# jfjlaros/HUMID

Measured on AMD Instinct MI355X. Metric: reads/sec deduplicated, 10M PE150 UMI=8 d=1, higher is better.
Workload: dtype u64; 1 GPU; 10000000 reads/GPU x 1 GPU (one shuffled read set of 10000000 reads, sliced by input order), PE150 UMI=8 in header -> 24-nt packed words (8+8+8), d=1, directional clustering; synthetic molecules=N/4, family 1+Geom(3), p_sub=1e-3, p_N=1e-4; reads_per_gpu=10000000, word_nt=24, distance=1, method=directional

## Files before the change

humid_amd/_lib.py:

```python
from __future__ import annotations

import ctypes as C
import os

_HERE = os.path.dirname(os.path.abspath(__file__))
SO_PATH = os.path.join(_HERE, "libhumid_hip.so")

u64p = C.POINTER(C.c_uint64)
u32p = C.POINTER(C.c_uint32)
u8p = C.POINTER(C.c_uint8)


class HumidSummary(C.Structure):
    _fields_ = [("total", C.c_uint64), ("usable", C.c_uint64), ("unique", C.c_uint64),
                ("clusters", C.c_uint64), ("edges", C.c_uint64), ("nonsingle", C.c_uint64),
                ("ms_count", C.c_float), ("ms_neighbours", C.c_float), ("ms_cluster", C.c_float),
                ("ms_map", C.c_float), ("ms_total", C.c_float), ("ms_h2d", C.c_float),
                ("ms_d2h", C.c_float), ("ms_k_insert", C.c_float), ("ms_k_pairs", C.c_float),
                ("ms_k_cluster", C.c_float), ("ms_k_map", C.c_float), ("ms_k_part", C.c_float),
                ("ms_k_unperm", C.c_float), ("count_mode_used", C.c_uint32)]

    def asdict(self):
        d = {k: getattr(self, k) for k, _ in self._fields_}
        d["records8"] = bool(d["count_mode_used"] >> 8)
        d["count_mode_used"] &= 0xff
        return d


class HumidConsensusSummary(C.Structure):
    _fields_ = [(k, C.c_uint64) for k in ("n_clusters", "total_bytes", "multi_read", "bases_changed", "votes", "errors")]

    def asdict(self):
        return {k: int(getattr(self, k)) for k, _ in self._fields_}


HOST_ALL_GATHER_FN = C.CFUNCTYPE(C.c_int, C.c_void_p, C.c_void_p, C.c_uint64, C.c_void_p)
EXCHANGE_FN = C.CFUNCTYPE(C.c_int, C.c_void_p, C.c_void_p, u64p, u64p, C.c_void_p, u64p, u64p, C.c_int, C.c_void_p)


class HumidComm(C.Structure):
    _fields_ = [("user", C.c_void_p), ("rank", C.c_uint32), ("world", C.c_uint32),
                ("host_all_gather", HOST_ALL_GATHER_FN), ("exchange", EXCHANGE_FN)]


class HumidExchangeInfo(C.Structure):
    _fields_ = [("unique_local", C.c_uint64), ("id_base", C.c_uint64), ("n_nodes", C.c_uint64),
                ("n_pairs", C.c_uint64), ("d_unique_count", C.c_void_p), ("d_unique_degree", C.c_void_p)]
# ... 168 lines not shown
```

humid_amd/csrc/humid_hip.hip:

```cpp
#include "pipeline.hip.h"
#include "kernels_best.hip.h"
#include "kernels_consensus.hip.h"

static std::string g_err;
extern "C" __attribute__((visibility("hidden"))) void humid_set_global_error(const char *text) { g_err = text ? text : ""; }

extern "C" {

uint32_t humid_abi_version(void) { return HUMID_ABI_VERSION; }

int humid_device_count(void) {
  int n = 0;
  if (hipGetDeviceCount(&n) != hipSuccess) return 0;
  return n;
}

const char *humid_last_error(const humid_ctx *ctx) { return ctx ? ctx->err.c_str() : g_err.c_str(); }

int humid_ctx_create(humid_ctx **out, int device, void *stream) {
  humid_ctx *c = nullptr;
  if (!out) return fail(nullptr, HUMID_E_INVALID, "out is null");
  *out = nullptr;
  int ndev = 0;
  hipError_t e = hipGetDeviceCount(&ndev);
// ... 126 lines not shown
  }
  if (strcmp(key, "kernel_timing") == 0) {
    c->kev_on = value != 0;
    return HUMID_OK;
  }
  if (strcmp(key, "test_fail_before_gather") == 0) {
    c->x_test_fail_after = (int)value;
    return HUMID_OK;
  }
  if (strcmp(key, "records8") == 0) {
    c->use_rec8 = value != 0;
    return HUMID_OK;
  }
  if (strcmp(key, "compact_graph") == 0) {
    c->use_compact = value != 0;
    return HUMID_OK;
  }
  if (strcmp(key, "group_buckets") == 0) {
    c->group_buckets = value != 0;
    return HUMID_OK;
  }
  if (strcmp(key, "fused_search") == 0) {
    c->fused_search = value != 0;
    return HUMID_OK;
  }
  if (strcmp(key, "padded_partition") == 0) {
    c->pt_padded = value != 0;
    return HUMID_OK;
  }
  if (strcmp(key, "force_comm") == 0) {
    c->force_comm = value != 0;
    return HUMID_OK;
  }
  if (strcmp(key, "bucket_walk") == 0) {
    if (value < 0 || value > (1 << 24)) return fail(c, HUMID_E_INVALID, "bucket_walk must be 0 (no limit) .. 2^24");
    c->walk_max = (u32)value;
    return HUMID_OK;
  }
  if (strcmp(key, "plan_segments") == 0) {
    if (value < 0 || value > 32) return fail(c, HUMID_E_INVALID, "plan_segments must be 0 (auto) .. 32");
    c->force_segments = (u32)value;
    return HUMID_OK;
  }
  return fail(c, HUMID_E_INVALID, "unknown option '%s'", key);
}

// ... 816 lines not shown
```

humid_amd/csrc/kernels_cgraph.hip.h:

```cpp
#ifndef HUMID_KERNELS_CGRAPH_HIP_H
#define HUMID_KERNELS_CGRAPH_HIP_H

#include "common.hip.h"
#include "kernels_graph.hip.h"
#include "kernels_cluster.hip.h"

#define ER_REGIONS 64u
#define ER_STRIDE 32u
struct EdgeRegs {
  u64 *e;
  u32 cap_r;
  u32 *cur;
  const u64 *far;
  u32 n_far;
};
__device__ __forceinline__ u32 er_count(const EdgeRegs &er, u32 r) {
  if (r == ER_REGIONS) return er.n_far;
  const u32 c = er.cur[r * ER_STRIDE];
  return c < er.cap_r ? c : er.cap_r;
}
__device__ __forceinline__ u64 *er_at(const EdgeRegs &er, u32 r, u32 k) {
  return r == ER_REGIONS ? (u64 *)er.far + k : er.e + (size_t)r * er.cap_r + k;
}

// ... 61 lines not shown
template <class WT>
struct WordsGlobal {
  const WT *W;
  __device__ __forceinline__ WT operator()(u32 j) const { return W[j]; }
};
struct IdxSelf { __device__ __forceinline__ u32 operator()(u32 j) const { return j; } };
struct IdxGlobal {
  const u32 *V;
  __device__ __forceinline__ u32 operator()(u32 j) const { return V[j]; }
};
template <class WT>
struct PairRule {
  WT mask;
  EarlierMasksT<WT> em;
  u32 cb, distance, walk_max;
};
template <class WT>
__device__ __forceinline__ bool pa_pair(WT x, const PairRule<WT> &r) {
  if (w_mismatch(x) > r.distance) return false;
  for (u32 t = 0; t < r.cb; t++)
    if (!w_hits(x, r.em.m[t])) return false;
  return true;
}
__device__ __forceinline__ u32 pa_jend(u32 i, u32 n, u32 walk_max) { return (walk_max && n - i > walk_max + 1) ? i + walk_max + 1 : n; }
template <class WT, class ACC>
__device__ __forceinline__ void pa_walk(const ACC &word, WT wi, WT w1, u32 i, u32 n, const PairRule<WT> &r, ull *big, u32 &found, u32 &first_off) {
  const u32 jend = pa_jend(i, n, r.walk_max);
  u32 j = i + 1;
  for (; j < jend; j++) {
    const WT x = w_xor(wi, j == i + 1 ? w1 : word(j));
    if (w_hits(x, r.mask)) break;
    if (!pa_pair(x, r)) continue;
    if (!found) first_off = j - i;
    found++;
  }
  if (big && j == jend && jend < n && !w_hits(w_xor(wi, word(jend)), r.mask)) atomicOr(big, 1ull << r.cb);
}
template <u32 NP, u32 NW, class WT, class ACC, class IDX>
__device__ __forceinline__ void pa_emit(const ACC &word, const IDX &idx, u32 i0, u32 stride, u32 n, const u32 (&found)[NP],
                                        const u32 (&first_off)[NP], const PairRule<WT> &r, const EdgeRegs &er, u32 *bits, u32 *overflow,
                                        u32 *lds) {
  u32 total_found = 0;
#pragma unroll
  for (u32 q = 0; q < NP; q++) total_found += found[q];
  const u32 lane = threadIdx.x & 63, wv = threadIdx.x >> 6;
  const u32 incl = wave_incl_scan(total_found);
  if (lane == 63) lds[wv] = incl;
  __syncthreads();
  u32 before = 0, total = 0;
#pragma unroll
  for (u32 k = 0; k < NW; k++) { const u32 x = lds[k]; if (k < wv) before += x; total += x; }
  if (total == 0) return;
  const u32 region = blockIdx.x % ER_REGIONS;
  if (threadIdx.x == 0) lds[NW] = atomicAdd(&er.cur[region * ER_STRIDE], total);
  __syncthreads();
  if (!total_found) return;
  u32 at = lds[NW] + before + incl - total_found;
  if (at + total_found > er.cap_r) { *overflow = 1; if (at >= er.cap_r) return; }
  u64 *out = er.e + (size_t)region * er.cap_r;
#pragma unroll
  for (u32 q = 0; q < NP; q++) {
    if (!found[q]) continue;
    const u32 i = i0 + q * stride;
    const u32 ri = idx(i);
    auto emit = [&](u32 j) {
      if (at >= er.cap_r) return;
      const u32 rj = idx(j);
      out[at++] = ri < rj ? (((u64)ri << 32) | rj) : (((u64)rj << 32) | ri);
      atomicOr(&bits[rj >> 5], 1u << (rj & 31));
    };
    atomicOr(&bits[ri >> 5], 1u << (ri & 31));
    if (found[q] == 1) { emit(i + first_off[q]); continue; }
    const WT wi = word(i);
    const u32 jend = pa_jend(i, n, r.walk_max);
    for (u32 j = i + first_off[q]; j < jend; j++) {
      const WT x = w_xor(wi, word(j));
      if (w_hits(x, r.mask)) break;
      if (pa_pair(x, r)) emit(j);
    }
  }
}
// ... 41 lines not shown
  const u32 *v_in;
  __device__ __forceinline__ u32 operator()(u32 j) const { return v_in[inv[j]]; }
};
struct PairSearchDev {
  static constexpr bool on = true;
  PairRule<u64> rule;
  EdgeRegs er;
  u32 *bits;
  ull *big;
  u32 *overflow;
  template <u32 NP, u32 T>
  __device__ __forceinline__ void in_bin(const u64 *sw, u32 n, const unsigned short *inv, const u32 *v_in, u32 *scratch) const {
    const WordsLds word{sw};
    u32 found[NP], first_off[NP];
#pragma unroll
    for (u32 q = 0; q < NP; q++) {
      const u32 i = threadIdx.x + q * T;
      found[q] = 0; first_off[q] = 0;
      if (i < n) pa_walk(word, sw[i], sw[i + 1 < n ? i + 1 : i], i, n, rule, big, found[q], first_off[q]);
    }
    pa_emit<NP, T / 64u>(word, IdxGrouped{inv, v_in}, threadIdx.x, T, n, found, first_off, rule, er, bits, overflow, scratch);
  }
};

static __global__ void __launch_bounds__(256)
k_mark_pairs(const u64 *__restrict__ pairs, u32 n_pairs, u32 n_leaves, u32 *bits, u32 *bad) {
  HUMID_GUARD_LAST_VGPR();
  const u32 k = blockIdx.x * blockDim.x + threadIdx.x;
  if (k >= n_pairs) return;
  const u64 e = pairs[k];
  const u32 a = (u32)(e >> 32), b = (u32)e;
  if (a >= n_leaves || b >= n_leaves || a == b) { *bad = 1; return; }
  atomicOr(&bits[a >> 5], 1u << (a & 31));
  atomicOr(&bits[b >> 5], 1u << (b & 31));
}

static __global__ void __launch_bounds__(256)
k_nodes_init(BitRank br, u32 n_words, const u32 *__restrict__ s_cnt, u32 *__restrict__ nodes, u32 *__restrict__ ncnt,
             u32 *__restrict__ deg, u32 *__restrict__ parent, u32 *__restrict__ csize, u32 *__restrict__ cur, u32 n_blk) {
  HUMID_GUARD_LAST_VGPR();
  const u32 w = blockIdx.x * blockDim.x + threadIdx.x;
  if (w == 0) deg[br.blk[n_blk]] = 0;
  if (w >= n_words) return;
  u32 x = br.bits[w];
  if (!x) return;
  u32 c = br_rank(br, w << 5);
// ... 246 lines not shown
```

humid_amd/csrc/kernels_part8.hip.h:

```cpp
#ifndef HUMID_KERNELS_PART8_HIP_H
#define HUMID_KERNELS_PART8_HIP_H

#include "common.hip.h"
#include "kernels_count.hip.h"
#include "kernels_part.hip.h"

#define P8_CAP2_LOG 10u
#define P8_CAP2 (1u << P8_CAP2_LOG)
#define P8_RPT (P8_CAP2 / 256u)

struct RecKey {
  u64 lo, scale;
  u32 z, kbits;
  u32 pow2;
  __host__ __device__ __forceinline__ u64 operator()(u64 w) const { return ((w - lo) * scale) >> z; }
  __device__ __forceinline__ u64 word(u64 k) const {
    if (pow2) return lo + k;
    const u64 x = k << z, q = x / scale;
    return lo + q + ((x - q * scale) ? 1u : 0u);
  }
};

struct Reads8 {
  const u64 *words;
// ... 154 lines not shown
  else {
    u32 ww = w;
    start = w << 5;
    while (ww > 0) {
      const u32 pz = ~lbits[ww - 1];
      if (pz) { start = ((ww - 1) << 5) + (32u - (u32)__clz((int)pz)); break; }
      ww--;
      start = ww << 5;
    }
  }
  const u32 za = bit < 31 ? (~bw & ~((2u << bit) - 1u)) : 0u;
  if (za) end = (w << 5) + (u32)__ffs((int)za) - 1u;
  else {
    u32 ww = w + 1;
    while (true) {
      const u32 nz = ~lbits[ww];
      if (nz) { end = (ww << 5) + (u32)__ffs((int)nz) - 1u; break; }
      ww++;
    }
  }
}
#define DR_WORDS (DR_SLOTS / 32u)
#define DR_EARLY 1u
static __global__ void __launch_bounds__(256)
k_dedup_rec(u64 *recs, const u32 *__restrict__ cursor2, u32 n_reads, u32 pb, u32 d1, u32 ibits, RecKey rk,
            u64 *__restrict__ pad_word, uint2 *__restrict__ pad_cf, u64 *__restrict__ agg, ull *ctr) {
  HUMID_GUARD_LAST_VGPR();
  PH_DECL;
  __shared__ u64 lkey[DR_SLOTS];
  __shared__ uint2 lcf[DR_SLOTS];
  __shared__ unsigned short lslot_of[P8_CAP2];
  __shared__ u32 lbits[DR_WORDS + 2], lpre[DR_WORDS + 2];
  __shared__ u32 lcount;
  const u32 g = blockIdx.x;
  const size_t beg = (size_t)g << P8_CAP2_LOG;
  PH(0);
  u64 rq[P8_RPT];
#pragma unroll
  for (u32 q = 0; q < DR_EARLY; q++) rq[q] = recs[beg + threadIdx.x + 256u * q];
  u32 n = cursor2[g];
  if (n > P8_CAP2) n = P8_CAP2;
  if (n == 0) {
    if (threadIdx.x == 0) agg[g] = 0;
    return;
  }
#pragma unroll
  for (u32 q = DR_EARLY; q < P8_RPT; q++) {
    const u32 i = threadIdx.x + 256u * q;
    if (i < n) rq[q] = recs[beg + i];
// ... 27 lines not shown
      if (++s >= DR_SLOTS) break;
    }
    if (s >= DR_SLOTS) { bad = true; continue; }
    sq[q] = s;
    atomicAdd(&lcf[s].x, 1u);
    atomicMin(&lcf[s].y, v);
    if (claimed) {
      lslot_of[atomicAdd(&lcount, 1u)] = (unsigned short)s;
      atomicOr(&lbits[s >> 5], 1u << (s & 31));
    }
  }
  if (bad) ctr[CTR_OVERFULL] = 1;
  PH(2);
  __syncthreads();
  PH(3);
  const u32 n_uniq = lcount;
  const u32 lane = threadIdx.x & 63;
  if ((threadIdx.x & ~63u) < n_uniq) {
    const u32 pc = lane < DR_WORDS ? (u32)__popc(lbits[lane]) : 0u;
    u32 incl = pc;
    incl = wave_incl_scan(incl);
    if (lane < DR_WORDS) lpre[lane] = incl - pc;
  }
  for (u32 li = threadIdx.x; li < n_uniq; li += 256) {
    const u32 sl = lslot_of[li];
    const u32 w = sl >> 5, bit = sl & 31;
    const u32 bw = lbits[w];
    u32 r = lpre[w] + (u32)__popc(bw & ((1u << bit) - 1u));
    const bool left = bit ? ((bw >> (bit - 1)) & 1u) != 0 : (w > 0 && (lbits[w - 1] >> 31) != 0);
    const bool right = bit < 31 ? ((bw >> (bit + 1)) & 1u) != 0 : (lbits[w + 1] & 1u) != 0;
    const u64 k = lkey[sl];
    if (left || right) {
      u32 start, end, smaller = 0;
      dr_run_bounds(lbits, w, bit, bw, start, end);
      if (end > DR_SLOTS) end = DR_SLOTS;
      for (u32 j = start; j < end; j++) smaller += lkey[j] < k ? 1u : 0u;
      r = r - (sl - start) + smaller;
    }
    const uint2 cf = lcf[sl];
    pad_word[beg + r] = rk.word(k);
    pad_cf[beg + r] = cf;
    lcf[sl].y = r;
  }
  if (threadIdx.x == 0) agg[g] = ((u64)n << 32) | n_uniq;
  PH(4);
  __syncthreads();
  PH(5);
#pragma unroll
  for (u32 q = 0; q < P8_RPT; q++) {
    const u32 i = threadIdx.x + 256u * q;
    if (i >= n) continue;
    const u32 li = sq[q] != NONE32 ? lcf[sq[q]].y : NONE32;
    recs[beg + i] = ((u64)(li < n ? (u32)beg + li : NOSLOT) << 32) | (u32)(rq[q] & imask);
  }
  PH(6);
  PH_END(0, 6, (g & 255u) == 77u);
}

static __global__ void __launch_bounds__(256)
k_compact_padded8(const u64 *__restrict__ pad_word, const uint2 *__restrict__ pad_cf, const u64 *__restrict__ agg,
                  const u64 *__restrict__ abase, u32 n_parts, u64 *__restrict__ s_word, u32 *__restrict__ s_slot,
                  u32 *__restrict__ s_cnt, u32 *__restrict__ s_first) {
  HUMID_GUARD_LAST_VGPR();
  const u32 wave = (blockIdx.x * blockDim.x + threadIdx.x) >> 6;
  const u32 lane = threadIdx.x & 63;
  if (wave >= n_parts) return;
  const u32 beg = wave << P8_CAP2_LOG, uc = (u32)agg[wave], ub = (u32)abase[wave];
  for (u32 j = lane; j < uc; j += 64) {
    s_word[ub + j] = pad_word[beg + j];
    s_slot[ub + j] = beg + j;
    const uint2 cf = pad_cf[beg + j];
    s_cnt[ub + j] = cf.x;
    s_first[ub + j] = cf.y;
  }
}

template <u32 NBMAX, u32 UIPT = 8u>
__global__ void __launch_bounds__(1024, NBMAX <= 1536 ? 8 : 4)
k_unperm_bins8(const u64 *__restrict__ recs, const u32 *__restrict__ cursor2, const u64 *__restrict__ slot_out, u32 n_parts,
// ... 330 lines not shown
```

humid_amd/csrc/pipeline.hip.h:

```cpp
#ifndef HUMID_PIPELINE_HIP_H
#define HUMID_PIPELINE_HIP_H

#include <fcntl.h>
#include <sys/mman.h>
#include <sys/stat.h>
#include <unistd.h>

#include <atomic>
#include <cerrno>
#include <chrono>
#include <type_traits>
#include <utility>

#include "common.hip.h"
#include "prims.hip.h"
#include "kernels_count.hip.h"
#include "kernels_part.hip.h"
#include "kernels_part8.hip.h"
#include "kernels_graph.hip.h"
#include "kernels_cluster.hip.h"
#include "kernels_cgraph.hip.h"
#include "kernels_map.hip.h"
#include "kernels_xchg.hip.h"
#include "kernels_wide.hip.h"
// ... 89 lines not shown
  DBuf xr_hist, xr_recv, xr_eloc, xr_got, xr_eall, xr_ret;
  DBuf x_slot, x_slot_s, x_cnt, x_cnts, x_rec, x_ncnt, x_route, x_creator, x_base, x_mark, x_markcr, x_scan, x_lcid, x_lismax,
       x_items, x_w, x_id, x_ids, x_ends, x_ends_s, x_head, x_hpos, x_nodes, x_cedges;
  DBuf w_sorted, w_head, w_hpos, w_start, w_heads;
  DBuf cg_edges, cg_cur, cg_far, cg_bits, cg_nbits, cg_blk, cg_nblk, cg_nodes, cg_ncnt, cg_deg, cg_off, cg_idx, cg_parent, cg_csize,
       cg_curs, cg_cl_of, cg_maxleaf, cg_cl_size;
  u64 cg_ecap = 0;
  bool use_compact = true;
  bool cg_valid = false;
  bool cg_expanded = false;
  u32 cg_M = 0, cg_nblocks = 0;
  DBuf xo_gw, xo_gc;
  DBuf xo_regs, xo_inv;
  u64 xr_ecap = 0;
  DBuf xo_send, xo_int, xo_cross, xo_sel, xo_selall, xo_parent, xo_flag, xo_xroot, xo_xcbits, xo_xcblk, xo_xcid, xo_xcall, xo_ldeg, xo_cnt;
  DBuf pw_a, pw_ai, pw_b, pw_bi;
  DBuf p8_a, p8_b, p8_cur, p8_status;
  bool use_rec8 = true;
  bool last_rec8 = false;
  const u32 *rec_cursor2 = nullptr;
  DBuf pt_work, unperm_rec, route_tiles;
  bool group_buckets = true;
  bool fused_search = true;
  bool pt_padded = true;
  bool use_tile_partition = true;
  bool last_part_tiled = false;
  int x_test_fail_after = -1, x_gathers = 0;
  bool x_hist_done = false, x_peer_failed = false;
  bool route_checked = true;
  const u32 *route_bad = nullptr;
  bool last_unperm_tiled = false;
  bool oc_valid = false, oc_fits = false;
  u32 oc_n = 0, oc_nt = 0;
  u64 oc_lo = 0, oc_scale = 0;
  u32 n_parts = 0;
  bool stage_map_timed = false;
  bool last_count_sorted = false;
  u32 g_wpr = 1;
  bool slots_done = false;
  int count_mode = 0;
  u32 force_segments = 0;
  bool force_comm = false;
  u32 walk_max = PT2_TILE;
  bool coop_big = true;
  bool last_count_lds = false;
  bool last_count_ordered = false;
// ... 577 lines not shown
  rk.lo = km.lo; rk.scale = km.scale;
  rk.pow2 = km.shift < 64 ? 1u : 0u;
  rk.z = rk.pow2 ? km.shift : 63u - (u32)__builtin_clzll(km.scale);
  rk.kbits = 64 - rk.z;
  const u32 ibits = bits_for(N);
  u32 d1 = (pb + 1) / 2;
  while (d1 < 10 && pb - d1 > 1 && rk.kbits - d1 + ibits > 64) d1++;
  const u32 d2 = pb - d1, nb1 = 1u << d1, n_parts = 1u << pb;
  if (rk.kbits < pb + 1 || rk.kbits - d1 + ibits > 64 || d2 > 9 || d2 == 0) return HUMID_OK;
  static const u32 pad_div = getenv("HUMID_PAD_DIV") ? (u32)std::max(1, atoi(getenv("HUMID_PAD_DIV"))) : 4u;
  const u32 cap1 = (u32)std::min<u64>(0xffffffffull / nb1, (u64)N / nb1 + (u64)N / nb1 / pad_div + 1024);
  const size_t room1 = (size_t)nb1 * cap1, room2 = (size_t)n_parts << P8_CAP2_LOG;
  ENSURE(c->p8_a, room1 * 8);
  ENSURE(c->p8_b, room2 * 8);
  ENSURE(c->pad_word, room2 * 8);
  ENSURE(c->pad_cf, room2 * 8);
  ENSURE(c->slot_out, (room2 + 1) * 8);
  ENSURE(c->pbeg, (size_t)(n_parts + 1) * 4);
  ENSURE(c->ucount, (size_t)(n_parts + 1) * 4);
  ENSURE(c->p8_status, ((size_t)n_parts + 1) * 16);
  u64 *agg = c->p8_status.as<u64>(), *abase = agg + n_parts + 1;
  ENSURE(c->p8_cur, ((size_t)PT_MAXBINS1 + n_parts + 2 * (PT_MAXBINS1 + 1)) * 4);
  u32 *cursor1 = c->p8_cur.as<u32>(), *cursor2 = cursor1 + PT_MAXBINS1, *cbase = cursor2 + n_parts, *tprefix = cbase + PT_MAXBINS1 + 1;
  HIPCHK(hipEventRecord(c->ev[0], st));
  {
    ZeroList z;
    memset(&z, 0, sizeof z);
    z.p[0] = cursor1; z.n[0] = PT_MAXBINS1 + n_parts;
    z.p[1] = (u32 *)c->d_ctr; z.n[1] = 2 * CTR_N;
    z.p[2] = (u32 *)(agg + n_parts); z.n[2] = 2;
    hipLaunchKernelGGL(k_zero_many, dim3(32), dim3(256), 0, st, z);
  }
  const bool check_range = !(range_lo == 0 && range_hi == ~0ull);
  const Reads8 src{d_words, d_filt, range_lo, range_hi, check_range ? 1u : 0u, rk};
  const u32 tiles1 = (N + PT_TILE - 1) / PT_TILE, tiles2 = tiles1 + nb1;
  static const bool s1_small = getenv("HUMID_S1_THREADS") ? atoi(getenv("HUMID_S1_THREADS")) == 512 : false;
  if (s1_small && nb1 <= 512)
    hipLaunchKernelGGL((k_p8_scatter1<Reads8, 512>), dim3((N + 4095) / 4096), dim3(512), 0, st, src, N, rk.kbits, d1, ibits, cap1, cursor1,
                       c->p8_a.as<u64>(), c->d_ctr);
  else
    hipLaunchKernelGGL((k_p8_scatter1<Reads8, 1024>), dim3(tiles1), dim3(1024), 0, st, src, N, rk.kbits, d1, ibits, cap1, cursor1,
                       c->p8_a.as<u64>(), c->d_ctr);
  hipLaunchKernelGGL(k_pt_scan1, dim3(1), dim3(1024), 0, st, (const u32 *)cursor1, d1, d2, cbase, tprefix, c->pbeg.as<u32>(),
                     c->ucount.as<u32>() + n_parts, cap1);
  if (c->kev_on) HIPCHK(hipEventRecord(c->kev[39], st));
  hipLaunchKernelGGL(k_p8_scatter2, dim3(tiles2), dim3(1024), 0, st, (const u64 *)c->p8_a.as<u64>(), (const u32 *)tprefix,
                     (const u32 *)cbase, rk.kbits, d1, d2, ibits, cap1, cursor2, c->p8_b.as<u64>(), c->d_ctr);
  if (c->kev_on) HIPCHK(hipEventRecord(c->kev[40], st));
  HIPCHK(hipEventRecord(c->kev[0], st));
  hipLaunchKernelGGL(k_dedup_rec, dim3(n_parts), dim3(256), 0, st, c->p8_b.as<u64>(), (const u32 *)cursor2, N, pb, d1, ibits, rk,
                     c->pad_word.as<u64>(), c->pad_cf.as<uint2>(), agg, c->d_ctr);
  HIPCHK(hipEventRecord(c->kev[1], st));
  TRY(exscan_in<u64>(c, PtrIn<u64>{agg}, abase, (u64)n_parts + 1));
  ENSURE(c->s_word, (size_t)(N + 1) * 8);
  ENSURE(c->s_slot, (size_t)(N + 1) * 4);
  ENSURE(c->s_cnt, (size_t)(N + 1) * 4);
  ENSURE(c->s_first, (size_t)(N + 1) * 4);
  hipLaunchKernelGGL(k_compact_padded8, dim3(blocks_for((u64)n_parts * 64)), dim3(256), 0, st, c->pad_word.as<u64>(),
                     c->pad_cf.as<uint2>(), (const u64 *)agg, (const u64 *)abase, n_parts, c->s_word.as<u64>(),
                     c->s_slot.as<u32>(), c->s_cnt.as<u32>(), c->s_first.as<u32>());
  if (!c->lean_events) HIPCHK(hipEventRecord(c->ev[1], st));
  HIPCHK(hipGetLastError());
  TRY(read_counters(c, (const u32 *)(abase + n_parts), (const u32 *)(abase + n_parts) + 1));
  if (getenv("HUMID_TRACE_COUNT"))
    fprintf(stderr, "[rec count] N %u pb %u kbits %u ibits %u cap1 %u special %llu overfull %llu unique %llu usable %llu\n", N, pb, rk.kbits,
            ibits, cap1, (ull)c->h_ctr[CTR_SPECIAL], (ull)c->h_ctr[CTR_OVERFULL], (ull)(c->h_ctr[CTR_N - 1] & 0xffffffffull), (ull)(c->h_ctr[CTR_N - 2] & 0xffffffffull));
  if (c->h_ctr[CTR_SPECIAL]) { c->pt_padded = false; return HUMID_OK; }
  if (c->h_ctr[CTR_OVERFULL]) return HUMID_OK;
  c->last_count_lds = true;
  c->last_count_sorted = false;
  c->last_count_ordered = true;
  c->last_part_tiled = true;
  c->last_rec8 = true;
  c->rec_cursor2 = cursor2;
  c->n_parts = n_parts;
  const u32 U = (u32)(c->h_ctr[CTR_N - 1] & 0xffffffffull);
  s.usable = c->usable = c->h_ctr[CTR_N - 2] & 0xffffffffull;
  s.unique = c->U = U;
  *done = true;
  return HUMID_OK;
}

static int stage_count_rec_wide(humid_ctx *c, const W2 *d_words, const u8 *d_filt, u32 N, u32 word_nt, const KeyMap &km,
                                humid_summary &s, bool *done) {
  hipStream_t st = c->stream;
  *done = false;
  if (!c->use_rec8 || !c->use_tile_partition || !c->pt_padded) return HUMID_OK;
  const u32 pb = part_bits(N);
  if (pb < 6 || pb > 18) return HUMID_OK;
  if ((((u64)N + (1u << UW_MAXSHIFT) - 1) >> UW_MAXSHIFT) > UW_MAXBINS) return HUMID_OK;
  const u32 d1 = (pb + 1) / 2, d2 = pb - d1, nb1 = 1u << d1, n_parts = 1u << pb;
  RecKey rk;
  rk.lo = km.lo; rk.scale = km.scale;
  rk.pow2 = km.shift < 64 ? 1u : 0u;
  rk.z = rk.pow2 ? km.shift : 63u - (u32)__builtin_clzll(km.scale);
  rk.kbits = 64 - rk.z;
  if (rk.kbits < pb + 1) return HUMID_OK;
  const u32 hbits = 2 * (word_nt - 32);
// ... 94 lines not shown
  double worst = 0;
  if (pb >= bits) {
    u32 mx = 0;
    for (u32 v : h) if (v > mx) mx = v;
    worst = (double)mx / (double)(1u << (pb - bits));
  } else {
    const u32 per = 1u << (bits - pb);
    for (u32 b = 0; b < n_bins; b += per) {
      u64 t = 0;
      for (u32 k = 0; k < per; k++) t += h[b + k];
      if ((double)t > worst) worst = (double)t;
    }
  }
  worst *= (double)N / (double)n_sample;
  *fits = worst * 1.5 <= (double)LDS_FILL_LIMIT;
  c->oc_valid = true; c->oc_fits = *fits;
  c->oc_n = N; c->oc_nt = word_nt; c->oc_lo = km.lo; c->oc_scale = km.scale;
  return HUMID_OK;
}

static int stage_count(humid_ctx *c, const u64 *d_words, const u8 *d_filt, u32 N, u32 word_nt,
                       u64 range_lo, u64 range_hi, u64 expected_reads, humid_summary &s, bool within = false) {
  const bool full_range = (range_lo == 0 && range_hi == ~0ull);
  if (c->count_mode == 0 && (full_range || within)) {
    const KeyMap km = key_map(word_nt, range_lo, range_hi, within);
    bool overflowed = false;
    bool ordered = c->count_order == 1;
    if (c->count_order < 0) TRY(prefix_fits_ordered(c, d_words, d_filt, N, word_nt, km, &ordered));
    c->last_rec8 = false;
    if (ordered) {
      bool done = false;
      TRY(stage_count_rec(c, d_words, d_filt, N, word_nt, range_lo, range_hi, km, s, &done));
      if (done) return HUMID_OK;
      TRY(stage_count_lds(c, d_words, d_filt, N, word_nt, range_lo, range_hi, km, true, s, &overflowed));
      if (!overflowed) return HUMID_OK;
      c->oc_valid = true; c->oc_fits = false;
      c->oc_n = N; c->oc_nt = word_nt; c->oc_lo = km.lo; c->oc_scale = km.scale;
    }
    TRY(stage_count_lds(c, d_words, d_filt, N, word_nt, range_lo, range_hi, km, false, s, &overflowed));
    if (!overflowed) return HUMID_OK;
  }
  return stage_count_global(c, d_words, d_filt, N, word_nt, range_lo, range_hi, expected_reads, s);
}

static int stage_count_wide(humid_ctx *c, const W2 *d_words, const u8 *d_filt, u32 N, u32 word_nt, humid_summary &s,
                            u64 head_lo = 0, u64 head_hi = ~0ull, bool within = false) {
// ... 580 lines not shown
  return HUMID_OK;
}

template <class WT>
static int stage_graph_compact(humid_ctx *c, const WT *g_word, const u32 *g_cnt, u32 U, u32 word_nt,
                               u32 distance, u32 method, humid_summary &s, u32 &n_pair_segs_out,
                               const u64 *ext_edges = nullptr, u64 n_ext_edges = 0) {
  hipStream_t st = c->stream;
  c->g_word = g_word;
  c->g_wpr = (u32)(sizeof(WT) / 8);
  c->g_cnt = g_cnt;
  c->gU = U;
  c->cg_valid = false;
  c->cg_expanded = false;
  const ComboPlan plan = make_plan(word_nt - c->gk_nt, distance, U, c->force_segments, true, c->gk_nt);
  const PairSearch<WT> ps = pair_search<WT>(c, plan, distance);
  const bool given = ext_edges != nullptr;
  const bool search = !given && distance > 0 && U > 1;
  if (search && plan.ncombo == 1 && plan.key_bits == 0 && U > (1u << 18))
    return fail(c, HUMID_E_OVERFLOW, "distance %u over %u-nt words compares all pairs of %u unique words: too many neighbour pairs",
                distance, word_nt, U);
  if (given && n_ext_edges > 0x7fffffffull) return fail(c, HUMID_E_OVERFLOW, "too many neighbour pairs");
  const u32 nseg = search ? plan.ncombo : 0;
  const u32 n_words = (((U + 31) / 32) + 7) & ~7u, n_blk = n_words / 8;
  c->cg_nblocks = n_blk;
  ENSURE(c->cg_bits, (size_t)n_words * 4);
  ENSURE(c->cg_nbits, (size_t)n_words * 4);
  ENSURE(c->cg_blk, ((size_t)n_blk + 1) * 4);
  ENSURE(c->cg_nblk, ((size_t)n_blk + 1) * 4);
  ENSURE(c->cg_cur, (size_t)(ER_REGIONS * ER_STRIDE + 8) * 4);
  ENSURE(c->small_roots, ((size_t)U / 3 + 2) * 4);
  ENSURE(c->small, 64);
  TRY(ensure_seg_scratch<WT>(c, nseg, U));
  u32 *bad = c->cg_cur.as<u32>() + ER_REGIONS * ER_STRIDE;
  const u64 *far = given ? ext_edges : nullptr;
  u64 n_far = given ? n_ext_edges : 0;
  u64 E = 0, M = 0, Mbig = 0;
  CgStatus cgs;
  EdgeRegs er;
  bool ordered_seg[MAX_COMBOS] = {false};
  const u32 *seg_valid[MAX_COMBOS] = {nullptr};
  for (int attempt = 0;; attempt++) {
    if (attempt > 5) return fail(c, HUMID_E_INVALID, "internal: the pair list does not settle");
    if (search && c->cg_ecap == 0) c->cg_ecap = std::max<u64>((u64)U / 4, 4096);
    const u64 ecap = search ? c->cg_ecap : ER_REGIONS;
    if (ecap / ER_REGIONS + 1 > 0xfffffff0ull) return fail(c, HUMID_E_OVERFLOW, "too many neighbour pairs");
    er.cap_r = (u32)((ecap + ER_REGIONS - 1) / ER_REGIONS);
    ENSURE(c->cg_edges, (size_t)ER_REGIONS * er.cap_r * 8);
    er.e = c->cg_edges.as<u64>();
    er.cur = c->cg_cur.as<u32>();
    er.far = far;
    er.n_far = (u32)n_far;
    {
      ZeroList z;
      memset(&z, 0, sizeof z);
      z.p[0] = c->cg_bits.as<u32>(); z.n[0] = n_words;
      z.p[1] = c->cg_nbits.as<u32>(); z.n[1] = n_words;
      z.p[2] = c->cg_cur.as<u32>(); z.n[2] = ER_REGIONS * ER_STRIDE + 8;
      z.p[3] = (u32 *)&c->d_ctr[CTR_EDGES]; z.n[3] = 2 * (CTR_GOVER - CTR_EDGES + 1);
      hipLaunchKernelGGL(k_zero_many, dim3(64), dim3(256), 0, st, z);
    }
    auto search_alone = [&](u32 seg) -> int {
      if (seg < 8 && c->kev_on) HIPCHK(hipEventRecord(c->kev[20 + 2 * seg], st));
      pairs_append<WT>(c, ps, walked_seg<WT>(c, plan, seg, g_word, U), er, c->cg_bits.as<u32>(), &c->d_ctr[CTR_BIGMASK],
                       (u32 *)&c->d_ctr[CTR_EOVER], seg_valid[seg]);
      if (seg < 8 && c->kev_on) HIPCHK(hipEventRecord(c->kev[21 + 2 * seg], st));
      return HUMID_OK;
    };
    const bool ride_on = c->fused_search && std::is_same<WT, u64>::value;
    for (u32 seg = 0; seg < nseg; seg++) {
      bool searched = false;
      if (seg) {
        seg_valid[seg] = nullptr;
        if (!ordered_seg[seg]) {
          GroupRide ride;
          if constexpr (std::is_same<WT, u64>::value) {
            if (ride_on) {
              ride.group = pairs_append_dev(ps, w_from<u64>(plan.mask[seg]), seg, er, c->cg_bits.as<u32>(), &c->d_ctr[CTR_BIGMASK], (u32 *)&c->d_ctr[CTR_EOVER]);
              if (seg < 8 && c->kev_on) { ride.ev_group[0] = c->kev[20 + 2 * seg]; ride.ev_group[1] = c->kev[21 + 2 * seg]; }
            }
          }
          TRY(bucket_order<WT>(c, plan, seg, g_word, U, seg_ws<WT>(c, seg, U), seg_vs(c, seg, U), true, ride_on ? &ride : nullptr));
          seg_valid[seg] = c->gf_valid;
          searched = ride.did_group;
        }
        ordered_seg[seg] = true;
      }
      if (!searched) TRY(search_alone(seg));
    }
    if (n_far)
      hipLaunchKernelGGL(k_mark_pairs, dim3(blocks_for(n_far)), dim3(256), 0, st, far, (u32)n_far, U, c->cg_bits.as<u32>(), bad);
    CgSource src;
    src.er = er; src.recs = nullptr; src.n_recs = 0; src.cnt_by_id = g_cnt; src.n_ids = U;
    src.pairs_bound = ecap + n_far;
    TRY(cg_build(c, src, method, cgs));
    er = src.er;
    if (cgs.group_over) {
      c->gf_padded = false;
      for (u32 q = 0; q < MAX_COMBOS; q++) ordered_seg[q] = false;
      far = given ? ext_edges : nullptr;
      n_far = given ? n_ext_edges : 0;
      continue;
    }
    if (cgs.overflow) {
      c->cg_ecap = cgs.wanted + cgs.wanted / 2 + ER_REGIONS * 64;
      if (!given) { far = nullptr; n_far = 0; }
      continue;
    }
    if (given) {
      u32 h_bad = 0;
      HIPCHK(hipMemcpyAsync(&h_bad, bad, 4, hipMemcpyDeviceToHost, st));
// ... 387 lines not shown
template <class WT>
static int run_device(humid_ctx *c, const WT *d_words, const u8 *d_filt, u64 n_reads, u32 word_nt,
                      u32 distance, u32 method, u32 *d_cid, u8 *d_keep, humid_summary *sum) {
  if (!c) return HUMID_E_INVALID;
  constexpr bool WIDE = sizeof(WT) == 16;
  state_reset(c);
  TRY(check_run_args(c, n_reads, word_nt, method, 64));
  if (WIDE != (word_nt > 32)) return fail(c, HUMID_E_INVALID, "word layout does not match word_nt");
  if (WIDE && ((uintptr_t)d_words & 15)) return fail(c, HUMID_E_INVALID, "wide words must be 16-byte aligned on the device");
  if (n_reads && (!d_words || !d_filt || !d_cid || !d_keep)) return fail(c, HUMID_E_INVALID, "null buffer");
  HIPCHK(hipSetDevice(c->device));
  hipStream_t st = c->stream;
  const u32 N = (u32)n_reads;
  humid_summary s;
  memset(&s, 0, sizeof s);
  s.total = n_reads;
  c->last_unperm_tiled = false;
  c->N = n_reads; c->U = c->E = c->M = c->C = c->usable = 0;
  c->word_nt = word_nt; c->distance = distance; c->method = method;
  c->gU = 0;
  if (N == 0) { if (sum) *sum = s; return state_publish(c, CtxState::RUN); }
  struct LeanEvents { humid_ctx *c; ~LeanEvents() { c->lean_events = false; } } lean_guard{c};
  c->lean_events = !c->kev_on && getenv("HUMID_ALL_EVENTS") == nullptr;
  if constexpr (WIDE) TRY(stage_count_wide(c, d_words, d_filt, N, word_nt, s));
  else TRY(stage_count(c, d_words, d_filt, N, word_nt, 0ull, ~0ull, 0, s));
  TRY(gkey_check(c));
  const u32 U = (u32)c->U;
  if (U == 0) {
    HIPCHK(hipMemsetAsync(d_cid, 0, (size_t)N * 4, st));
    HIPCHK(hipMemsetAsync(d_keep, 0, (size_t)N, st));
    HIPCHK(hipStreamSynchronize(st));
    if (sum) *sum = s;
    return state_publish(c, CtxState::RUN);
  }
  u32 n_pair_segs = 0;
  if (c->edit && distance >= 2) {
    u64 E = 0;
    TRY(edit_edges<WT>(c, c->s_word.as<WT>(), U, word_nt, distance, &E));
    static const u64 no_edges = 0;
    if (c->use_compact)
      TRY(stage_graph_compact<WT>(c, c->s_word.as<WT>(), c->s_cnt.as<u32>(), U, word_nt, distance, method, s, n_pair_segs,
                                  E ? c->e_edges.as<u64>() : &no_edges, E));
    else
      TRY(stage_graph<WT>(c, c->s_word.as<WT>(), c->s_cnt.as<u32>(), U, word_nt, distance, method, s, n_pair_segs,
                          E ? c->e_edges.as<u64>() : &no_edges, E));
  } else if (c->use_compact)
    TRY(stage_graph_compact<WT>(c, c->s_word.as<WT>(), c->s_cnt.as<u32>(), U, word_nt, distance, method, s, n_pair_segs));
  else
    TRY(stage_graph<WT>(c, c->s_word.as<WT>(), c->s_cnt.as<u32>(), U, word_nt, distance, method, s, n_pair_segs));
  TRY(stage_map(c, c->cid.as<u32>(), c->ismax.as<u8>(), N, d_cid, d_keep));
  if (c->cg_valid) TRY(n_clusters_compact(c, U, &c->C));
  else TRY(n_clusters_from_scan(c, U, &c->C));
  s.clusters = c->C;
  const u64 E = c->E, M = c->M;
  HIPCHK(hipEventSynchronize(c->ev[4]));
  const bool lean = c->lean_events;
  c->lean_events = false;
  if (!lean) {
    HIPCHK(hipEventElapsedTime(&s.ms_count, c->ev[0], c->ev[1]));
    HIPCHK(hipEventElapsedTime(&s.ms_neighbours, c->ev[1], c->ev[2]));
    HIPCHK(hipEventElapsedTime(&s.ms_cluster, c->ev[2], c->ev[3]));
    HIPCHK(hipEventElapsedTime(&s.ms_map, c->ev[3], c->ev[4]));
  }
  HIPCHK(hipEventElapsedTime(&s.ms_total, c->ev[0], c->ev[4]));
  TRY(gkey_check(c));
  HIPCHK(hipEventElapsedTime(&s.ms_k_insert, c->kev[0], c->kev[1]));
  if (!c->kev_on) s.ms_k_map = s.ms_map;
  else if (c->last_count_lds) HIPCHK(hipEventElapsedTime(&s.ms_k_map, c->ev[3], c->kev[36]));
  else s.ms_k_map = s.ms_map;
  if (c->kev_on && c->last_count_lds && c->last_unperm_tiled) HIPCHK(hipEventElapsedTime(&s.ms_k_unperm, c->kev[36], c->kev[41]));
  if (c->kev_on && c->last_count_lds && c->last_part_tiled && !c->last_count_sorted) HIPCHK(hipEventElapsedTime(&s.ms_k_part, c->kev[39], c->kev[40]));
  s.count_mode_used = (c->last_count_sorted ? 3u : c->last_count_lds ? (c->last_count_ordered ? 2u : 0u) : 1u) | (c->last_rec8 ? 0x100u : 0u);
  if (c->kev_on) HIPCHK(hipEventElapsedTime(&s.ms_k_cluster, c->kev[2], c->kev[3]));
  for (u32 g = 0; c->kev_on && g < n_pair_segs; g++) {
    float t = 0;
    HIPCHK(hipEventElapsedTime(&t, c->kev[20 + 2 * g], c->kev[21 + 2 * g]));
    s.ms_k_pairs += t;
    if (E > 0 && !c->cg_valid) {
      HIPCHK(hipEventElapsedTime(&t, c->kev[4 + 2 * g], c->kev[5 + 2 * g]));
      s.ms_k_pairs += t;
    }
  }
  if (sum) *sum = s;
  return state_publish(c, CtxState::RUN);
}

static inline u32 gkey_nt_for(u32 n_groups) { return n_groups <= 1 ? 0u : (bits_for(n_groups) + 1) / 2; }

static int check_grouped_args(humid_ctx *c, u32 word_nt, u32 n_groups) {
  if (n_groups == 0) return fail(c, HUMID_E_INVALID, "n_groups must be >= 1");
  if (word_nt >= 1 && word_nt <= 64 && word_nt + gkey_nt_for(n_groups) > 64)
    return fail(c, HUMID_E_UNSUPPORTED, "word_nt %u + %u group nucleotides (%u groups) > 64 is not supported", word_nt,
                gkey_nt_for(n_groups), n_groups);
  return HUMID_OK;
}
// ... 157 lines not shown
```

Before: 16.66 billion reads/s.

## Fuse first-segment neighbour search into dedup kernel via per-bucket rooms

Adds a prefix-search mode, on by default. The bucketed dedup kernel reorders its LDS keys by rank and, while the bucket is still resident in LDS, walks segment 0's neighbour pairs and writes them into fixed-size per-bucket rooms. A small k_pairs_rooms kernel then turns those compact local pairs into global edges and marks the leaf bits, replacing the separate segment-0 search pass over the global sorted words. This trades a re-read of global words for extra LDS work and barriers inside the dedup kernel. A room capacity of 128 pairs falls back to the old path on overflow, and the shape of the last run is cached to decide whether to try again.

Result: slower. 16.26 billion reads/s (-2.4%).

```diff
diff --git a/humid_amd/_lib.py b/humid_amd/_lib.py
--- a/humid_amd/_lib.py
+++ b/humid_amd/_lib.py
@@ -22,7 +22,8 @@
 
     def asdict(self):
         d = {k: getattr(self, k) for k, _ in self._fields_}
-        d["records8"] = bool(d["count_mode_used"] >> 8)
+        d["records8"] = bool(d["count_mode_used"] >> 8 & 1)
+        d["prefix_search"] = bool(d["count_mode_used"] >> 9 & 1)
         d["count_mode_used"] &= 0xff
         return d
 
diff --git a/humid_amd/csrc/humid_hip.hip b/humid_amd/csrc/humid_hip.hip
--- a/humid_amd/csrc/humid_hip.hip
+++ b/humid_amd/csrc/humid_hip.hip
@@ -172,6 +172,10 @@
   }
   if (strcmp(key, "fused_search") == 0) {
     c->fused_search = value != 0;
+    return HUMID_OK;
+  }
+  if (strcmp(key, "prefix_search") == 0) {
+    c->prefix_search = value != 0;
     return HUMID_OK;
   }
   if (strcmp(key, "padded_partition") == 0) {
diff --git a/humid_amd/csrc/kernels_cgraph.hip.h b/humid_amd/csrc/kernels_cgraph.hip.h
--- a/humid_amd/csrc/kernels_cgraph.hip.h
+++ b/humid_amd/csrc/kernels_cgraph.hip.h
@@ -107,9 +107,15 @@
     if (!w_hits(x, r.em.m[t])) return false;
   return true;
 }
+struct PrefixRule {
+  u64 mask;
+  u32 distance, walk_max;
+  static constexpr u32 cb = 0;
+};
+__device__ __forceinline__ bool pa_pair(u64 x, const PrefixRule &r) { return w_mismatch(x) <= r.distance; }
 __device__ __forceinline__ u32 pa_jend(u32 i, u32 n, u32 walk_max) { return (walk_max && n - i > walk_max + 1) ? i + walk_max + 1 : n; }
-template <class WT, class ACC>
-__device__ __forceinline__ void pa_walk(const ACC &word, WT wi, WT w1, u32 i, u32 n, const PairRule<WT> &r, ull *big, u32 &found, u32 &first_off) {
+template <class WT, class ACC, class RULE>
+__device__ __forceinline__ void pa_walk(const ACC &word, WT wi, WT w1, u32 i, u32 n, const RULE &r, ull *big, u32 &found, u32 &first_off) {
   const u32 jend = pa_jend(i, n, r.walk_max);
   u32 j = i + 1;
   for (; j < jend; j++) {
@@ -121,6 +127,24 @@
   }
   if (big && j == jend && jend < n && !w_hits(w_xor(wi, word(jend)), r.mask)) atomicOr(big, 1ull << r.cb);
 }
+template <u32 NW>
+__device__ __forceinline__ bool pa_reserve(u32 total_found, const EdgeRegs &er, u32 *overflow, u32 *lds, u32 &region, u32 &at) {
+  const u32 lane = threadIdx.x & 63, wv = threadIdx.x >> 6;
+  const u32 incl = wave_incl_scan(total_found);
+  if (lane == 63) lds[wv] = incl;
+  __syncthreads();
+  u32 before = 0, total = 0;
+#pragma unroll
+  for (u32 k = 0; k < NW; k++) { const u32 x = lds[k]; if (k < wv) before += x; total += x; }
+  if (total == 0) return false;
+  region = blockIdx.x % ER_REGIONS;
+  if (threadIdx.x == 0) lds[NW] = atomicAdd(&er.cur[region * ER_STRIDE], total);
+  __syncthreads();
+  if (!total_found) return false;
+  at = lds[NW] + before + incl - total_found;
+  if (at + total_found > er.cap_r) { *overflow = 1; if (at >= er.cap_r) return false; }
+  return true;
+}
 template <u32 NP, u32 NW, class WT, class ACC, class IDX>
 __device__ __forceinline__ void pa_emit(const ACC &word, const IDX &idx, u32 i0, u32 stride, u32 n, const u32 (&found)[NP],
                                         const u32 (&first_off)[NP], const PairRule<WT> &r, const EdgeRegs &er, u32 *bits, u32 *overflow,
@@ -128,20 +152,8 @@
   u32 total_found = 0;
 #pragma unroll
   for (u32 q = 0; q < NP; q++) total_found += found[q];
-  const u32 lane = threadIdx.x & 63, wv = threadIdx.x >> 6;
-  const u32 incl = wave_incl_scan(total_found);
-  if (lane == 63) lds[wv] = incl;
-  __syncthreads();
-  u32 before = 0, total = 0;
-#pragma unroll
-  for (u32 k = 0; k < NW; k++) { const u32 x = lds[k]; if (k < wv) before += x; total += x; }
-  if (total == 0) return;
-  const u32 region = blockIdx.x % ER_REGIONS;
-  if (threadIdx.x == 0) lds[NW] = atomicAdd(&er.cur[region * ER_STRIDE], total);
-  __syncthreads();
-  if (!total_found) return;
-  u32 at = lds[NW] + before + incl - total_found;
-  if (at + total_found > er.cap_r) { *overflow = 1; if (at >= er.cap_r) return; }
+  u32 region, at;
+  if (!pa_reserve<NW>(total_found, er, overflow, lds, region, at)) return;
   u64 *out = er.e + (size_t)region * er.cap_r;
 #pragma unroll
   for (u32 q = 0; q < NP; q++) {
@@ -229,6 +241,81 @@
     pa_emit<NP, T / 64u>(word, IdxGrouped{inv, v_in}, threadIdx.x, T, n, found, first_off, rule, er, bits, overflow, scratch);
   }
 };
+
+struct WordsRanked {
+  const u64 *lkey;
+  RecKey rk;
+  __device__ __forceinline__ u64 operator()(u32 j) const { return rk.word(lkey[j]); }
+};
+struct PrefixSearchDev {
+  static constexpr bool on = true;
+  u64 mask;
+  u32 distance, walk_max;
+  u32 *count;
+  u32 *room;
+  ull *big;
+  u32 *over;
+  __device__ __forceinline__ void in_bucket(const u64 *lkey, u32 n, const RecKey &rk, u32 g, u32 *lcnt) const {
+    const WordsRanked word{lkey, rk};
+    const PrefixRule rule{mask, distance, walk_max};
+    u32 *out = room + ((size_t)g << PR_CAP_LOG);
+    for (u32 i = threadIdx.x; i < n; i += 256u) {
+      u32 found = 0, first_off = 0;
+      const u64 wi = word(i);
+      pa_walk(word, wi, word(i + 1 < n ? i + 1 : i), i, n, rule, big, found, first_off);
+      if (!found) continue;
+      u32 at = atomicAdd(lcnt, found);
+      atomicAdd(&count[g], found);
+      if (at + found > PR_CAP) *over = 1;
+      auto emit = [&](u32 j) { if (at < PR_CAP) out[at] = i << 16 | j; at++; };
+      if (found == 1) { emit(i + first_off); continue; }
+      const u32 jend = pa_jend(i, n, walk_max);
+      for (u32 j = i + first_off; j < jend; j++) {
+        const u64 x = wi ^ word(j);
+        if (w_hits(x, mask)) break;
+        if (pa_pair(x, rule)) emit(j);
+      }
+    }
+  }
+};
+static __global__ void __launch_bounds__(256)
+k_pairs_rooms(const u32 *__restrict__ count, const u32 *__restrict__ room, const u64 *__restrict__ abase, u32 n_parts,
+              const ull *__restrict__ big_seen, EdgeRegs er, u32 *bits, ull *big, u32 *overflow) {
+  HUMID_GUARD_LAST_VGPR();
+  __shared__ u32 lds[5];
+  if (blockIdx.x == 0 && threadIdx.x == 0) {
+    const ull b = *big_seen;
+    if (b) atomicOr(big, b);
+  }
+  const u32 g = blockIdx.x * 32u + (threadIdx.x >> 3), e0 = (threadIdx.x & 7u) * 4u;
+  u32 cnt = 0, nf = 0, ub = 0;
+  uint4 ent = make_uint4(0u, 0u, 0u, 0u);
+  const u32 *mine = room + ((size_t)g << PR_CAP_LOG);
+  if (g < n_parts) {
+    cnt = count[g];
+    if (cnt > PR_CAP) cnt = PR_CAP;
+    if (e0 < cnt) {
+      ent = *(const uint4 *)(mine + e0);
+      ub = (u32)abase[g];
+      for (u32 e = e0; e < cnt; e += 32u) nf += cnt - e < 4u ? cnt - e : 4u;
+    }
+  }
+  u32 region, at;
+  if (!pa_reserve<4>(nf, er, overflow, lds, region, at)) return;
+  u64 *out = er.e + (size_t)region * er.cap_r;
+  for (u32 e = e0; e < cnt; e += 32u) {
+    if (e != e0) ent = *(const uint4 *)(mine + e);
+    const u32 v[4] = {ent.x, ent.y, ent.z, ent.w};
+#pragma unroll
+    for (u32 q = 0; q < 4; q++) {
+      if (e + q >= cnt || at >= er.cap_r) break;
+      const u32 ri = ub + (v[q] >> 16), rj = ub + (v[q] & 0xffffu);
+      out[at++] = ((u64)ri << 32) | rj;
+      atomicOr(&bits[ri >> 5], 1u << (ri & 31));
+      atomicOr(&bits[rj >> 5], 1u << (rj & 31));
+    }
+  }
+}
 
 static __global__ void __launch_bounds__(256)
 k_mark_pairs(const u64 *__restrict__ pairs, u32 n_pairs, u32 n_leaves, u32 *bits, u32 *bad) {
diff --git a/humid_amd/csrc/kernels_part8.hip.h b/humid_amd/csrc/kernels_part8.hip.h
--- a/humid_amd/csrc/kernels_part8.hip.h
+++ b/humid_amd/csrc/kernels_part8.hip.h
@@ -200,9 +200,14 @@
 }
 #define DR_WORDS (DR_SLOTS / 32u)
 #define DR_EARLY 1u
-static __global__ void __launch_bounds__(256)
+struct NoPrefixSearch { static constexpr bool on = false; };
+__device__ __forceinline__ void lds_barrier() { asm volatile("s_waitcnt lgkmcnt(0)\n\ts_barrier" ::: "memory"); }
+#define PR_CAP_LOG 7u
+#define PR_CAP (1u << PR_CAP_LOG)
+template <class SEARCH = NoPrefixSearch>
+__global__ void __launch_bounds__(256)
 k_dedup_rec(u64 *recs, const u32 *__restrict__ cursor2, u32 n_reads, u32 pb, u32 d1, u32 ibits, RecKey rk,
-            u64 *__restrict__ pad_word, uint2 *__restrict__ pad_cf, u64 *__restrict__ agg, ull *ctr) {
+            u64 *__restrict__ pad_word, uint2 *__restrict__ pad_cf, u64 *__restrict__ agg, ull *ctr, SEARCH srch = SEARCH()) {
   HUMID_GUARD_LAST_VGPR();
   PH_DECL;
   __shared__ u64 lkey[DR_SLOTS];
@@ -276,6 +281,8 @@
     incl = wave_incl_scan(incl);
     if (lane < DR_WORDS) lpre[lane] = incl - pc;
   }
+  u64 k0 = 0;
+  u32 r0 = NONE32;
   for (u32 li = threadIdx.x; li < n_uniq; li += 256) {
     const u32 sl = lslot_of[li];
     const u32 w = sl >> 5, bit = sl & 31;
@@ -295,6 +302,7 @@
     pad_word[beg + r] = rk.word(k);
     pad_cf[beg + r] = cf;
     lcf[sl].y = r;
+    if constexpr (SEARCH::on) { if (li == threadIdx.x) { k0 = k; r0 = r; } }
   }
   if (threadIdx.x == 0) agg[g] = ((u64)n << 32) | n_uniq;
   PH(4);
@@ -308,7 +316,31 @@
     recs[beg + i] = ((u64)(li < n ? (u32)beg + li : NOSLOT) << 32) | (u32)(rq[q] & imask);
   }
   PH(6);
-  PH_END(0, 6, (g & 255u) == 77u);
+  if constexpr (SEARCH::on) {
+    if (threadIdx.x == 0) lcount = 0;
+    if (n_uniq > 256u) {
+      u64 kk[P8_RPT - 1];
+      u32 rr[P8_RPT - 1];
+#pragma unroll
+      for (u32 q = 1; q < P8_RPT; q++) {
+        const u32 li = threadIdx.x + 256u * q;
+        rr[q - 1] = NONE32;
+        if (li < n_uniq) { const u32 sl = lslot_of[li]; kk[q - 1] = lkey[sl]; rr[q - 1] = lcf[sl].y; }
+      }
+      lds_barrier();
+#pragma unroll
+      for (u32 q = 1; q < P8_RPT; q++)
+        if (rr[q - 1] < n_uniq) lkey[rr[q - 1]] = kk[q - 1];
+    }
+    if (r0 < n_uniq) lkey[r0] = k0;
+    lds_barrier();
+    PH(7);
+    srch.in_bucket(lkey, n_uniq, rk, g, &lcount);
+    PH(8);
+    PH_END(0, 8, (g & 255u) == 77u);
+  } else {
+    PH_END(0, 6, (g & 255u) == 77u);
+  }
 }
 
 static __global__ void __launch_bounds__(256)
diff --git a/humid_amd/csrc/pipeline.hip.h b/humid_amd/csrc/pipeline.hip.h
--- a/humid_amd/csrc/pipeline.hip.h
+++ b/humid_amd/csrc/pipeline.hip.h
@@ -135,6 +135,12 @@
   DBuf pt_work, unperm_rec, route_tiles;
   bool group_buckets = true;
   bool fused_search = true;
+  bool prefix_search = true;
+  DBuf pr_rooms;
+  struct PrefixHint { bool on = false; u32 distance = 0, walk_max = 0; u64 mask = 0; } pr_hint;
+  struct PrefixRooms { bool valid = false, over = false; u32 distance = 0, walk_max = 0, n_parts = 0; u64 mask = 0; } pr;
+  struct PrefixShape { bool known = false, off = false; u32 N = 0, word_nt = 0, distance = 0, gk_nt = 0, force_segments = 0, U = 0; } pr_shape;
+  bool last_prefix_rooms = false;
   bool pt_padded = true;
   bool use_tile_partition = true;
   bool last_part_tiled = false;
@@ -758,6 +764,17 @@
   u64 *agg = c->p8_status.as<u64>(), *abase = agg + n_parts + 1;
   ENSURE(c->p8_cur, ((size_t)PT_MAXBINS1 + n_parts + 2 * (PT_MAXBINS1 + 1)) * 4);
   u32 *cursor1 = c->p8_cur.as<u32>(), *cursor2 = cursor1 + PT_MAXBINS1, *cbase = cursor2 + n_parts, *tprefix = cbase + PT_MAXBINS1 + 1;
+  const humid_ctx::PrefixHint hint = c->pr_hint;
+  bool ride = false;
+  if (hint.on && hint.mask && rk.pow2 && rk.lo == 0 && rk.kbits == 2 * word_nt) {
+    const u32 tz = (u32)__builtin_ctzll(hint.mask), L = (u32)__builtin_popcountll(hint.mask);
+    ride = (hint.mask >> tz) == (L == 64 ? ~0ull : (1ull << L) - 1ull) && tz + L == rk.kbits && L >= pb;
+  }
+  u32 *pr_room = nullptr, *pr_count = nullptr, *pr_flags = nullptr;
+  if (ride) {
+    ENSURE(c->pr_rooms, (((size_t)n_parts << PR_CAP_LOG) + n_parts + 4) * 4);
+    pr_room = c->pr_rooms.as<u32>(); pr_count = pr_room + ((size_t)n_parts << PR_CAP_LOG); pr_flags = pr_count + n_parts;
+  }
   HIPCHK(hipEventRecord(c->ev[0], st));
   {
     ZeroList z;
@@ -765,6 +782,7 @@
     z.p[0] = cursor1; z.n[0] = PT_MAXBINS1 + n_parts;
     z.p[1] = (u32 *)c->d_ctr; z.n[1] = 2 * CTR_N;
     z.p[2] = (u32 *)(agg + n_parts); z.n[2] = 2;
+    if (ride) { z.p[3] = pr_count; z.n[3] = n_parts + 4; }
     hipLaunchKernelGGL(k_zero_many, dim3(32), dim3(256), 0, st, z);
   }
   const bool check_range = !(range_lo == 0 && range_hi == ~0ull);
@@ -784,8 +802,13 @@
                      (const u32 *)cbase, rk.kbits, d1, d2, ibits, cap1, cursor2, c->p8_b.as<u64>(), c->d_ctr);
   if (c->kev_on) HIPCHK(hipEventRecord(c->kev[40], st));
   HIPCHK(hipEventRecord(c->kev[0], st));
-  hipLaunchKernelGGL(k_dedup_rec, dim3(n_parts), dim3(256), 0, st, c->p8_b.as<u64>(), (const u32 *)cursor2, N, pb, d1, ibits, rk,
-                     c->pad_word.as<u64>(), c->pad_cf.as<uint2>(), agg, c->d_ctr);
+  if (ride)
+    hipLaunchKernelGGL(k_dedup_rec<PrefixSearchDev>, dim3(n_parts), dim3(256), 0, st, c->p8_b.as<u64>(), (const u32 *)cursor2, N, pb, d1, ibits,
+                       rk, c->pad_word.as<u64>(), c->pad_cf.as<uint2>(), agg, c->d_ctr,
+                       PrefixSearchDev{hint.mask, hint.distance, hint.walk_max, pr_count, pr_room, (ull *)pr_flags, pr_flags + 2});
+  else
+    hipLaunchKernelGGL(k_dedup_rec<NoPrefixSearch>, dim3(n_parts), dim3(256), 0, st, c->p8_b.as<u64>(), (const u32 *)cursor2, N, pb, d1, ibits,
+                       rk, c->pad_word.as<u64>(), c->pad_cf.as<uint2>(), agg, c->d_ctr, NoPrefixSearch{});
   HIPCHK(hipEventRecord(c->kev[1], st));
   TRY(exscan_in<u64>(c, PtrIn<u64>{agg}, abase, (u64)n_parts + 1));
   ENSURE(c->s_word, (size_t)(N + 1) * 8);
@@ -797,7 +820,7 @@
                      c->s_slot.as<u32>(), c->s_cnt.as<u32>(), c->s_first.as<u32>());
   if (!c->lean_events) HIPCHK(hipEventRecord(c->ev[1], st));
   HIPCHK(hipGetLastError());
-  TRY(read_counters(c, (const u32 *)(abase + n_parts), (const u32 *)(abase + n_parts) + 1));
+  TRY(read_counters(c, (const u32 *)(abase + n_parts), (const u32 *)(abase + n_parts) + 1, ride ? pr_flags + 2 : nullptr));
   if (getenv("HUMID_TRACE_COUNT"))
     fprintf(stderr, "[rec count] N %u pb %u kbits %u ibits %u cap1 %u special %llu overfull %llu unique %llu usable %llu\n", N, pb, rk.kbits,
             ibits, cap1, (ull)c->h_ctr[CTR_SPECIAL], (ull)c->h_ctr[CTR_OVERFULL], (ull)(c->h_ctr[CTR_N - 1] & 0xffffffffull), (ull)(c->h_ctr[CTR_N - 2] & 0xffffffffull));
@@ -810,6 +833,10 @@
   c->last_rec8 = true;
   c->rec_cursor2 = cursor2;
   c->n_parts = n_parts;
+  if (ride) {
+    c->pr.valid = true; c->pr.over = (c->h_ctr[CTR_N - 3] & 0xffffffffull) != 0;
+    c->pr.distance = hint.distance; c->pr.walk_max = hint.walk_max; c->pr.n_parts = n_parts; c->pr.mask = hint.mask;
+  }
   const u32 U = (u32)(c->h_ctr[CTR_N - 1] & 0xffffffffull);
   s.usable = c->usable = c->h_ctr[CTR_N - 2] & 0xffffffffull;
   s.unique = c->U = U;
@@ -950,6 +977,7 @@
 static int stage_count(humid_ctx *c, const u64 *d_words, const u8 *d_filt, u32 N, u32 word_nt,
                        u64 range_lo, u64 range_hi, u64 expected_reads, humid_summary &s, bool within = false) {
   const bool full_range = (range_lo == 0 && range_hi == ~0ull);
+  c->pr.valid = false;
   if (c->count_mode == 0 && (full_range || within)) {
     const KeyMap km = key_map(word_nt, range_lo, range_hi, within);
     bool overflowed = false;
@@ -1576,6 +1604,12 @@
                 distance, word_nt, U);
   if (given && n_ext_edges > 0x7fffffffull) return fail(c, HUMID_E_OVERFLOW, "too many neighbour pairs");
   const u32 nseg = search ? plan.ncombo : 0;
+  bool rooms = false;
+  if constexpr (std::is_same<WT, u64>::value)
+    rooms = search && c->pr.valid && !c->pr.over && (const void *)g_word == c->s_word.p && U == (u32)c->U && c->last_rec8 &&
+            c->pr.n_parts == c->n_parts && c->pr.mask == plan.mask[0].lo && plan.mask[0].hi == 0 && c->pr.walk_max == c->walk_max &&
+            c->pr.distance == distance;
+  c->last_prefix_rooms = rooms;
   const u32 n_words = (((U + 31) / 32) + 7) & ~7u, n_blk = n_words / 8;
   c->cg_nblocks = n_blk;
   ENSURE(c->cg_bits, (size_t)n_words * 4);
@@ -1621,6 +1655,15 @@
       if (seg < 8 && c->kev_on) HIPCHK(hipEventRecord(c->kev[21 + 2 * seg], st));
       return HUMID_OK;
     };
+    auto search_rooms = [&]() -> int {
+      if (c->kev_on) HIPCHK(hipEventRecord(c->kev[20], st));
+      const u32 np = c->pr.n_parts;
+      const u32 *room = c->pr_rooms.as<u32>(), *count = room + ((size_t)np << PR_CAP_LOG);
+      hipLaunchKernelGGL(k_pairs_rooms, dim3(blocks_for(np, 32)), dim3(256), 0, st, count, room, (const u64 *)c->p8_status.as<u64>() + np + 1, np,
+                         (const ull *)(count + np), er, c->cg_bits.as<u32>(), &c->d_ctr[CTR_BIGMASK], (u32 *)&c->d_ctr[CTR_EOVER]);
+      if (c->kev_on) HIPCHK(hipEventRecord(c->kev[21], st));
+      return HUMID_OK;
+    };
     const bool ride_on = c->fused_search && std::is_same<WT, u64>::value;
     for (u32 seg = 0; seg < nseg; seg++) {
       bool searched = false;
@@ -1640,7 +1683,7 @@
         }
         ordered_seg[seg] = true;
       }
-      if (!searched) TRY(search_alone(seg));
+      if (!searched) TRY(seg == 0 && rooms ? search_rooms() : search_alone(seg));
     }
     if (n_far)
       hipLaunchKernelGGL(k_mark_pairs, dim3(blocks_for(n_far)), dim3(256), 0, st, far, (u32)n_far, U, c->cg_bits.as<u32>(), bad);
@@ -2074,8 +2117,18 @@
   if (N == 0) { if (sum) *sum = s; return state_publish(c, CtxState::RUN); }
   struct LeanEvents { humid_ctx *c; ~LeanEvents() { c->lean_events = false; } } lean_guard{c};
   c->lean_events = !c->kev_on && getenv("HUMID_ALL_EVENTS") == nullptr;
+  struct PrefixGuard { humid_ctx *c; ~PrefixGuard() { c->pr_hint.on = false; c->pr.valid = false; } } prefix_guard{c};
+  c->pr_hint.on = false; c->pr.valid = false; c->pr.over = false; c->last_prefix_rooms = false;
+  const humid_ctx::PrefixShape sh = c->pr_shape;
+  const bool same_shape = sh.known && sh.N == N && sh.word_nt == word_nt && sh.distance == distance && sh.gk_nt == c->gk_nt &&
+                          sh.force_segments == c->force_segments;
+  if (!WIDE && c->prefix_search && c->use_compact && distance > 0 && !(c->edit && distance >= 2) && !(same_shape && sh.off)) {
+    const ComboPlan pred = make_plan(word_nt - c->gk_nt, distance, same_shape ? sh.U : N, c->force_segments, true, c->gk_nt);
+    if (pred.key_bits > 0 && pred.mask[0].hi == 0) c->pr_hint = humid_ctx::PrefixHint{true, distance, c->walk_max, pred.mask[0].lo};
+  }
   if constexpr (WIDE) TRY(stage_count_wide(c, d_words, d_filt, N, word_nt, s));
   else TRY(stage_count(c, d_words, d_filt, N, word_nt, 0ull, ~0ull, 0, s));
+  c->pr_hint.on = false;
   TRY(gkey_check(c));
   const u32 U = (u32)c->U;
   if (U == 0) {
@@ -2100,6 +2153,8 @@
     TRY(stage_graph_compact<WT>(c, c->s_word.as<WT>(), c->s_cnt.as<u32>(), U, word_nt, distance, method, s, n_pair_segs));
   else
     TRY(stage_graph<WT>(c, c->s_word.as<WT>(), c->s_cnt.as<u32>(), U, word_nt, distance, method, s, n_pair_segs));
+  c->pr_shape = humid_ctx::PrefixShape{true, (same_shape && sh.off) || (c->pr.valid && c->pr.over), N, word_nt, distance, c->gk_nt, c->force_segments, U};
+  c->pr.valid = false;
   TRY(stage_map(c, c->cid.as<u32>(), c->ismax.as<u8>(), N, d_cid, d_keep));
   if (c->cg_valid) TRY(n_clusters_compact(c, U, &c->C));
   else TRY(n_clusters_from_scan(c, U, &c->C));
@@ -2122,7 +2177,8 @@
   else s.ms_k_map = s.ms_map;
   if (c->kev_on && c->last_count_lds && c->last_unperm_tiled) HIPCHK(hipEventElapsedTime(&s.ms_k_unperm, c->kev[36], c->kev[41]));
   if (c->kev_on && c->last_count_lds && c->last_part_tiled && !c->last_count_sorted) HIPCHK(hipEventElapsedTime(&s.ms_k_part, c->kev[39], c->kev[40]));
-  s.count_mode_used = (c->last_count_sorted ? 3u : c->last_count_lds ? (c->last_count_ordered ? 2u : 0u) : 1u) | (c->last_rec8 ? 0x100u : 0u);
+  s.count_mode_used = (c->last_count_sorted ? 3u : c->last_count_lds ? (c->last_count_ordered ? 2u : 0u) : 1u) | (c->last_rec8 ? 0x100u : 0u) |
+                      (c->last_prefix_rooms ? 0x200u : 0u);
   if (c->kev_on) HIPCHK(hipEventElapsedTime(&s.ms_k_cluster, c->kev[2], c->kev[3]));
   for (u32 g = 0; c->kev_on && g < n_pair_segs; g++) {
     float t = 0;
```
